# potsawee/tokenize-audio

Hardware: AMD Instinct MI355X
Metric: audio-sec encoded/sec (Mimi 8-codebook, 24 kHz) (higher is better)
Workload: dtype f16x3 (fp32-emulating: 2 fp16 planes per operand, 3 products, fp32 accumulate; RVQ distances fp32); 1 GPU; LibriTTS-R-style batch encode (configs[1]): batch=32 x 10 s @ 24 kHz resident in HBM, K=8 codebooks, 1 encode per step per GPU; global_batch=32, num_quantizers=8, parallelism=utterance round-robin x1 (no collective), gemm_precision=f16x3

## Files before the change

tokenize-audio_amd/csrc/stage0_fused.hip:

```cpp
#include <type_traits>

#include "resblock_h16.h"

namespace mimi {

#ifndef S0F_HELP
#define S0F_HELP 1
#endif
#ifndef S0F_DIAG
#define S0F_DIAG 0
#endif
#if S0F_DIAG == 3
#define S0F_DRAIN() asm volatile("" ::: "memory")
#else
#define S0F_DRAIN() asm volatile("s_waitcnt lgkmcnt(0)" ::: "memory")
#endif
namespace s0f {
constexpr int NA = 4, NC = 8, NW = NA + NC;
constexpr int YLD = 72, YSR = 36, YSS = YSR * YLD + 16, YPS = 4 * YSS, YBS = 2 * YPS;
constexpr int OFF_SLAB = r0h::NFRAG * 1024 + r0h::BIAS * 4;
constexpr int OFF_Y = OFF_SLAB + NA * r0h::WAVE_BYTES;
constexpr int OFF_D = OFF_Y + 2 * YBS * 2;
constexpr int OFF_A2 = OFF_D + 2 * NA * 16 + 16;
constexpr int LDS_BYTES = OFF_A2 + (S0F_HELP ? NA * 2 * 2 * r0h::AUD * 2 : 0);
static_assert(OFF_SLAB % 16 == 0 && OFF_Y % 16 == 0 && (YSS * 2) % 16 == 0, "16-B alignment");
static_assert(LDS_BYTES <= 160 * 1024, "LDS");
static_assert(NC * 16 == 128, "conv waves x 16 channels = down conv 0's output channels");
}

#if S0F_STAMP
#define S0F_T0() unsigned long long st_last = __builtin_readcyclecounter(), st_acc[6] = {0, 0, 0, 0, 0, 0}
#define S0F_T(i)                                                  \
    do {                                                          \
        const unsigned long long now_ = __builtin_readcyclecounter(); \
        st_acc[i] += now_ - st_last;                              \
        st_last = now_;                                           \
    } while (0)
#define S0F_TPRINT(tag)                                                                                         \
    if (blockIdx.x == 0 && lane == 0 && R > 64)                                                                 \
    printf("s0f %s wave %d rounds %d: %llu %llu %llu %llu %llu %llu\n", tag, wave, R, st_acc[0], st_acc[1],     \
           st_acc[2], st_acc[3], st_acc[4], st_acc[5])
#else
#define S0F_T0()
#define S0F_T(i)
#define S0F_TPRINT(tag)
#endif
__global__ __launch_bounds__(768) void stage0_fused_h16_kernel(ResArgs p) {
    using namespace r0h;
    constexpr int YLD = s0f::YLD, YSS = s0f::YSS, YPS = s0f::YPS, YBS = s0f::YBS, NA = s0f::NA;
    __shared__ __attribute__((aligned(16))) char lds[s0f::LDS_BYTES];
    const int tid = threadIdx.x, lane = tid & 63;
    const int wave = __builtin_amdgcn_readfirstlane(tid >> 6);
    {
        const uint4* src = reinterpret_cast<const uint4*>(p.wh16);
        uint4* dst = reinterpret_cast<uint4*>(lds);
        for (int i = tid; i < NFRAG * 64; i += s0f::NW * 64) dst[i] = src[i];
        float* bw = reinterpret_cast<float*>(lds + NFRAG * 1024);
        if (tid < 64) {
            bw[tid] = p.b0[tid];
            bw[96 + tid] = p.b1[tid];
        }
        if (tid < 32) bw[64 + tid] = p.b3[tid];
    }
    _Float16* ybase = reinterpret_cast<_Float16*>(lds + s0f::OFF_Y);
    int4* desc = reinterpret_cast<int4*>(lds + s0f::OFF_D);
    int* rcount = reinterpret_cast<int*>(lds + s0f::OFF_D + 2 * NA * 16);

    const long long T = p.T;
    const unsigned tpi = (unsigned)((T + 31) >> 5);
    const unsigned long long NT = p.istart ? p.istart[p.batch] : (unsigned long long)tpi * p.batch;
    const unsigned long long NWT = (unsigned long long)gridDim.x * NA;
    auto range = [&](int w, unsigned& g0, unsigned& g1) {
        const unsigned long long wid = (unsigned long long)blockIdx.x * NA + w;
        g0 = (unsigned)(wid * NT / NWT);
        g1 = (unsigned)((wid + 1) * NT / NWT);
    };
    if (wave < NA) {
        unsigned g0, g1;
        range(wave, g0, g1);
        TileWalk tw(p, tpi, g0);
        if (lane == 0) {
            rcount[wave] = (int)(g1 - g0) + ((g0 < g1 && tw.t0 > 0) ? 1 : 0);
            desc[NA + wave] = make_int4(0, 0, 0, 0);
        }
    }
    __syncthreads();
    int R = 0;
#pragma unroll
    for (int w = 0; w < NA; ++w) R = max(R, rcount[w]);
    const __attribute__((address_space(1))) float* __restrict__ audio =
        (const __attribute__((address_space(1))) float*)io_pointer(p.audio_ref, p.audio);
    [[maybe_unused]] _Float16* aud2 = reinterpret_cast<_Float16*>(lds + s0f::OFF_A2);

    if (wave >= NA) {
        const int co0 = 16 * (wave - NA);
        const int c16 = lane & 15, kq = lane >> 4;
        f16x8 wr[16][2];
        {
            const _Float16* wd = reinterpret_cast<const _Float16*>(p.wdown);
#pragma unroll
            for (int s = 0; s < 16; ++s) {
                const int tap = (s >> 2) + 4 * (s & 1), lo = (s >> 1) & 1;
#pragma unroll
                for (int pl = 0; pl < 2; ++pl)
                    wr[s][pl] = *reinterpret_cast<const f16x8*>(wd + (long long)(pl * 128 + co0 + c16) * 512 + tap * 64 +
                                                                32 * lo + 8 * kq);
            }
        }
        const f32x4 bd = *reinterpret_cast<const f32x4*>(p.bdown + co0 + 4 * kq);
        const float ud = p.unscale_d;
        const int sec_l = (lane >> 3) & 1, rho = lane & 7;
#if S0F_HELP
        const int hw = (wave - NA) >> 1, hrole = (wave - NA) & 1;
        unsigned hg0, hg1;
        range(hw, hg0, hg1);
        TileWalk htw(p, tpi, hg0);
        const int hhs = (hg0 < hg1 && htw.t0 > 0) ? 1 : 0;
        htw.t0 -= 32 * hhs;
        const int hRw = (int)(hg1 - hg0) + hhs;
        float mxa = 0.0f;
        auto haload = [&]() {
            const long long pos = htw.t0 - 8 + lane;
            const bool ok = lane < AUD && pos >= 0 && pos < htw.Tb;
            const float v = audio[ok ? (long long)htw.b * T + pos : 0];
            return ok ? v : 0.0f;
        };
        auto hsplit = [&](int n, float av) {
            if (lane < AUD) {
                mxa = fmaxf(mxa, fabsf(av));
                unsigned hw_, lw_;
                split2_f16s(av, 0.0f, p.ascale, hw_, lw_);
                _Float16* im = aud2 + (hw * 2 + (n & 1)) * (2 * AUD);
                im[lane] = __builtin_bit_cast(f16x2, hw_)[0];
                im[AUD + lane] = __builtin_bit_cast(f16x2, lw_)[0];
            }
        };
        const int hrow_ = (lane >> 3) & 3;
        const int hoff_ = (lane >> 5) * YPS + hw * YSS + hrow_ * YLD + 8 * ((lane & 7) ^ ((hrow_ & 1) * 2));
        float hnext = 0.0f;
        if (hrole == 0 && hRw > 0) {
            hsplit(0, haload());
            htw.next();
            if (hRw > 1) hnext = haload();
        }
        __syncthreads();
#endif
        S0F_T0();
        for (int n = 0; n <= R; ++n) {
#if S0F_HELP
            if (hrole == 1 && n < hRw) {
                uint4 v = make_uint4(0u, 0u, 0u, 0u);
                if (htw.t0 > 0) v = *reinterpret_cast<const uint4*>(ybase + ((n + 1) & 1) * YBS + hoff_ + 32 * YLD);
                *reinterpret_cast<uint4*>(ybase + (n & 1) * YBS + hoff_) = v;
                htw.next();
            }
#endif
            if (n > 0) {
                const _Float16* yb = ybase + ((n + 1) & 1) * YBS;
                const int4* dsc = desc + ((n + 1) & 1) * NA;
                f32x4 acc[2];
#pragma unroll
                for (int i = 0; i < 2; ++i) acc[i] = (f32x4){0.0f, 0.0f, 0.0f, 0.0f};
#pragma unroll
                for (int s = 0; s < 16; ++s) {
                    const int tap = (s >> 2) + 4 * (s & 1), lo = (s >> 1) & 1;
                    const int row = 4 * rho + tap, ch = 4 * lo + kq;
                    const int o = row * YLD + 8 * (ch ^ ((row & 1) * 2));
                    f16x8 yf[2][2];
#pragma unroll
                    for (int i = 0; i < 2; ++i)
#pragma unroll
                        for (int pl = 0; pl < 2; ++pl)
                            yf[pl][i] = *reinterpret_cast<const f16x8*>(yb + pl * YPS + (2 * i + sec_l) * YSS + o);
#pragma unroll
                    for (int i = 0; i < 2; ++i) {
                        if (S0F_DIAG == 1) continue;
                        acc[i] = mfma_h16(wr[s][0], yf[1][i], acc[i]);
                        acc[i] = mfma_h16(wr[s][1], yf[0][i], acc[i]);
                        acc[i] = mfma_h16(wr[s][0], yf[0][i], acc[i]);
                    }
                }
                S0F_T(0);
#pragma unroll
                for (int i = 0; i < 2; ++i) {
                    const int4 d = dsc[2 * i + sec_l];
                    if (rho < d.z) {
                        f32x4 v;
#pragma unroll
                        for (int r = 0; r < 4; ++r) v[r] = acc[i][r] * ud + bd[r];
                        *reinterpret_cast<f32x4*>(p.xout + ((long long)d.x * p.T1 + d.y + rho) * 128 + co0 + 4 * kq) = v;
                    }
                }
                S0F_T(1);
            }
#if S0F_HELP
            if (hrole == 0 && n + 1 < hRw) {
                hsplit(n + 1, hnext);
                htw.next();
                if (n + 2 < hRw) hnext = haload();
            }
#endif
            __syncthreads();
            S0F_T(2);
        }
        S0F_TPRINT("conv");
#if S0F_HELP
        amax_commit(p.aamax, mxa);
#endif
        return;
    }

#ifdef S0F_PRIO
    __builtin_amdgcn_s_setprio(S0F_PRIO);
#endif
    const f16x8* wf = reinterpret_cast<const f16x8*>(lds);
    const float* bl = reinterpret_cast<const float*>(lds + NFRAG * 1024);
    _Float16* slab = reinterpret_cast<_Float16*>(lds + s0f::OFF_SLAB + wave * WAVE_BYTES);
    _Float16* hb = slab + 2 * SLD;
    float* aud = reinterpret_cast<float*>(slab + 2 * SPL);
    unsigned g0, g1;
    range(wave, g0, g1);
    TileWalk tw(p, tpi, g0);
    const int hstart = (g0 < g1 && tw.t0 > 0) ? 1 : 0;
    tw.t0 -= 32 * hstart;
    const int Rw = (int)(g1 - g0) + hstart;
    const int j = lane & 31, hh = lane >> 5;
    const float sa = p.ascale, sx = p.xscale, sh = p.hscale, sy = p.yscale;
    const float u0 = p.unscale0, u1 = p.unscale1, u2 = p.unscale2;
    float mxa = 0.0f, mxx = 0.0f, mxh = 0.0f, mxy = 0.0f;
    auto aload = [&](unsigned bb, long long t0) {
        const long long pos = t0 - 8 + lane;
        const bool ok = lane < AUD && pos >= 0 && pos < tw.Tb;
        const float v = audio[ok ? (long long)bb * T + pos : 0];
        return ok ? v : 0.0f;
    };
    _Float16* audh = reinterpret_cast<_Float16*>(aud);
    auto conv0_img = [&](const _Float16* img, f32x16 (&x0)[2]) {
        f16x8 bq;
        const _Float16* ap = img + (hh ? AUD : 0) + j + 2;
#pragma unroll
        for (int k = 0; k < 8; ++k) bq[k] = ap[k];
#pragma unroll
        for (int mt = 0; mt < 2; ++mt) {
            f32x16 acc;
#pragma unroll
            for (int r = 0; r < 16; ++r) acc[r] = 0.0f;
            acc = mfma_h(wf[(FR_W0 + 2 * mt + 1) * 64 + lane], bq, acc);
            acc = mfma_h(wf[(FR_W0 + 2 * mt) * 64 + lane], bq, acc);
#pragma unroll
            for (int g = 0; g < 4; ++g) {
                const f32x4 bb = *reinterpret_cast<const f32x4*>(bl + 32 * mt + 8 * g + 4 * hh);
#pragma unroll
                for (int q = 0; q < 4; ++q) x0[mt][4 * g + q] = __builtin_fmaf(acc[4 * g + q], u0, bb[q]);
            }
        }
    };
    auto conv0 = [&](float av, f32x16 (&x0)[2]) {
        if (lane < AUD) {
            mxa = fmaxf(mxa, fabsf(av));
            unsigned hw, lw;
            split2_f16s(av, 0.0f, sa, hw, lw);
            audh[lane] = __builtin_bit_cast(f16x2, hw)[0];
            audh[AUD + lane] = __builtin_bit_cast(f16x2, lw)[0];
        }
        S0F_DRAIN();
        conv0_img(audh, x0);
    };
    auto slab_put = [&](const f32x16 (&x0)[2], int rowoff) {
        const int row = j + rowoff;
        if (row < 0 || row >= SROWS) return;
#pragma unroll
        for (int mt = 0; mt < 2; ++mt)
#pragma unroll
            for (int g = 0; g < 4; ++g) {
                const float z[4] = {x0[mt][4 * g], x0[mt][4 * g + 1], x0[mt][4 * g + 2], x0[mt][4 * g + 3]};
                float t[4];
                elu_s4<true>(z, sx, t, mxx);
                uint2 hi, lo;
                split4_t(t, hi, lo);
                const int o = row * SLD + 32 * mt + 8 * g + 4 * hh;
                *reinterpret_cast<uint2*>(slab + o) = hi;
                *reinterpret_cast<uint2*>(slab + SPL + o) = lo;
            }
    };
    const int cpl = lane >> 5, crow = (lane >> 4) & 1, cc = (lane & 15) * 4;
    const int hrow = (lane >> 3) & 3;
    const int hoff = (lane >> 5) * YPS + wave * YSS + hrow * YLD + 8 * ((lane & 7) ^ ((hrow & 1) * 2));
    const int yrow = 4 + j, ysw = (yrow & 1) * 2;

    if (S0F_DIAG == 2) {
        for (int i = lane; i < YSS / 8; i += 64)
#pragma unroll
            for (int q = 0; q < 4; ++q)
                *reinterpret_cast<uint4*>(ybase + q * YPS + wave * YSS + 8 * i) = make_uint4(0u, 0u, 0u, 0u);
    }
#if S0F_HELP
    __syncthreads();
#else
    float anext = Rw > 0 ? aload(tw.b, tw.t0) : 0.0f;
#endif
    S0F_T0();
    for (int n = 0; n <= R; ++n) {
        _Float16* ycur = ybase + (n & 1) * YBS;
        const _Float16* yprev = ybase + ((n + 1) & 1) * YBS;
        int4* dcur = desc + (n & 1) * NA;
        if (n < Rw && S0F_DIAG == 2) {
            if (lane == 0) dcur[wave] = make_int4((int)tw.b, (int)(tw.t0 >> 2), n < hstart ? 0 : 1, 0);
            tw.next();
        } else if (n < Rw) {
            const unsigned b = tw.b;
            const long long t0 = tw.t0;
            const long long Tb = tw.Tb;
            if (!S0F_HELP) {
                uint4 v = make_uint4(0u, 0u, 0u, 0u);
                if (t0 > 0) v = *reinterpret_cast<const uint4*>(yprev + hoff + 32 * YLD);
                *reinterpret_cast<uint4*>(ycur + hoff) = v;
            }
            if (lane == 0) {
                const long long T1b = (Tb + 3) >> 2;
                const long long t10 = t0 >> 2;
                dcur[wave] = make_int4((int)b, (int)t10, n < hstart ? 0 : (int)min(8LL, T1b - t10), 0);
            }
            if (t0 == 0) {
                *reinterpret_cast<uint2*>(slab + cpl * SPL + crow * SLD + cc) = make_uint2(0u, 0u);
            } else if (n == 0) {
                f32x16 xp[2];
                conv0(aload(b, t0 - 32), xp);
                slab_put(xp, -30);
            }
            S0F_T(0);
            f32x16 x0[2];
#if S0F_HELP
            tw.next();
            conv0_img(aud2 + (wave * 2 + (n & 1)) * (2 * AUD), x0);
#else
            const float acur = anext;
            tw.next();
            anext = aload(tw.b, tw.t0);
            conv0(acur, x0);
#endif
            S0F_T(1);
            slab_put(x0, 2);
            S0F_DRAIN();
            S0F_T(2);

            f32x16 acc1;
#pragma unroll
            for (int r = 0; r < 16; ++r) acc1[r] = 0.0f;
            f16x8 fr[2][4];
            auto g1load = [&](int ks, f16x8 (&f)[4]) {
                const int o = (j + (ks >> 2)) * SLD + (ks & 3) * 16 + 8 * hh;
                f[0] = *reinterpret_cast<const f16x8*>(slab + o);
                f[1] = *reinterpret_cast<const f16x8*>(slab + SPL + o);
                f[2] = wf[(FR_W3 + 2 * ks) * 64 + lane];
                f[3] = wf[(FR_W3 + 2 * ks + 1) * 64 + lane];
            };
            g1load(0, fr[0]);
#pragma unroll
            for (int ks = 0; ks < 12; ++ks) {
                if (ks + 1 < 12) g1load(ks + 1, fr[(ks + 1) & 1]);
                const f16x8(&f)[4] = fr[ks & 1];
                acc1 = mfma_h(f[3], f[0], acc1);
                acc1 = mfma_h(f[2], f[1], acc1);
                acc1 = mfma_h(f[2], f[0], acc1);
            }
            {
                _Float16* sp = slab + cpl * SPL;
                const uint2 v = *reinterpret_cast<const uint2*>(sp + (32 + crow) * SLD + cc);
                *reinterpret_cast<uint2*>(sp + crow * SLD + cc) = v;
            }
            asm volatile("" ::: "memory");
#pragma unroll
            for (int gq = 0; gq < 4; ++gq) {
                const f32x4 bb = *reinterpret_cast<const f32x4*>(bl + 64 + 8 * gq + 4 * hh);
                float z[4], t[4];
#pragma unroll
                for (int q = 0; q < 4; ++q) z[q] = __builtin_fmaf(acc1[4 * gq + q], u1, bb[q]);
                elu_s4<true>(z, sh, t, mxh);
                uint2 hi, lo;
                split4_t(t, hi, lo);
                const int o = j * SLD + 8 * gq + 4 * hh;
                *reinterpret_cast<uint2*>(hb + o) = hi;
                *reinterpret_cast<uint2*>(hb + SPL + o) = lo;
            }
            S0F_DRAIN();
            S0F_T(3);

            f16x8 bh[2][2];
#pragma unroll
            for (int ks = 0; ks < 2; ++ks) {
                const int o = j * SLD + ks * 16 + 8 * hh;
                bh[ks][0] = *reinterpret_cast<const f16x8*>(hb + o);
                bh[ks][1] = *reinterpret_cast<const f16x8*>(hb + SPL + o);
            }
            float tmy = 0.0f;
            const bool yin = t0 + j < Tb;
            _Float16* ys = ycur + wave * YSS + yrow * YLD + 4 * hh;
#pragma unroll
            for (int mt = 0; mt < 2; ++mt) {
                f32x16 acc2;
#pragma unroll
                for (int r = 0; r < 16; ++r) acc2[r] = 0.0f;
#pragma unroll
                for (int ks = 0; ks < 2; ++ks) {
                    const f16x8 aw0 = wf[(FR_W1 + (mt * 2 + ks) * 2) * 64 + lane];
                    const f16x8 aw1 = wf[(FR_W1 + (mt * 2 + ks) * 2 + 1) * 64 + lane];
                    acc2 = mfma_h(aw1, bh[ks][0], acc2);
                    acc2 = mfma_h(aw0, bh[ks][1], acc2);
                    acc2 = mfma_h(aw0, bh[ks][0], acc2);
                }
#pragma unroll
                for (int gq = 0; gq < 4; ++gq) {
                    const f32x4 bb = *reinterpret_cast<const f32x4*>(bl + 96 + 32 * mt + 8 * gq + 4 * hh);
                    float z[4], t[4];
#pragma unroll
                    for (int q = 0; q < 4; ++q) z[q] = x0[mt][4 * gq + q] + __builtin_fmaf(acc2[4 * gq + q], u2, bb[q]);
                    elu_s4<true>(z, sy, t, tmy);
                    uint2 hi, lo;
                    split4_t(t, hi, lo);
                    if (!yin) hi = lo = make_uint2(0u, 0u);
                    const int o = 8 * ((4 * mt + gq) ^ ysw);
                    *reinterpret_cast<uint2*>(ys + o) = hi;
                    *reinterpret_cast<uint2*>(ys + YPS + o) = lo;
                    if (p.yp && yin) {
                        _Float16* g = reinterpret_cast<_Float16*>(p.yp) + ((long long)b * T + t0 + j) * 64 + 32 * mt +
                                      8 * gq + 4 * hh;
                        *reinterpret_cast<uint2*>(g) = hi;
                        *reinterpret_cast<uint2*>(g + p.y_pstride) = lo;
                    }
                }
            }
            if (yin) mxy = fmaxf(mxy, tmy);
            S0F_T(4);
        } else if (lane == 0) {
            dcur[wave] = make_int4(0, 0, 0, 0);
        }
        __syncthreads();
        S0F_T(5);
    }
    S0F_TPRINT("block");
    amax_commit(p.aamax, mxa);
    amax_commit(p.xamax, mxx * (1.0f / sx));
    amax_commit(p.hamax, mxh * (1.0f / sh));
    amax_commit(p.yamax, mxy * (1.0f / sy));
}

hipError_t launch_stage0_fused(const ResArgs& a, hipStream_t s, const char** kname) {
    if (a.T <= 0 || a.batch <= 0 || !a.audio || !a.wh16 || !a.wdown || !a.bdown || !a.xout ||
        a.T1 != (a.T + 3) / 4)
        return hipErrorInvalidValue;
    static const char* nm = "mimi::stage0_fused_h16_kernel(mimi::ResArgs)";
    if (kname) *kname = nm;
    int dev = 0, ncu = 256;
    (void)hipGetDevice(&dev);
    (void)hipDeviceGetAttribute(&ncu, hipDeviceAttributeMultiprocessorCount, dev);
    hipLaunchKernelGGL(stage0_fused_h16_kernel, dim3((unsigned)ncu), dim3(64 * s0f::NW), 0, s, a);
    return hipGetLastError();
}

}
```

Measured before the change: 56090 audio-sec/sec.

## Software-pipeline conv0 one tile ahead and template out optional tap stores

Helper waves now split audio two tiles ahead, and each block wave computes the next tile's conv0 MFMAs interleaved with the current tile's second GEMM, carrying the result across iterations. The aim is to hide conv0 latency and LDS load latency behind the existing MFMA chain. A template parameter removes the runtime yp tap-store branch when no taps are requested. The cost is more live registers (an extra x0 accumulator set) and an added barrier at startup.

```diff
diff --git a/tokenize-audio_amd/csrc/stage0_fused.hip b/tokenize-audio_amd/csrc/stage0_fused.hip
--- a/tokenize-audio_amd/csrc/stage0_fused.hip
+++ b/tokenize-audio_amd/csrc/stage0_fused.hip
@@ -6,6 +6,16 @@
 
 #ifndef S0F_HELP
 #define S0F_HELP 1
+#endif
+#ifndef S0F_AHEAD
+#define S0F_AHEAD 1
+#endif
+#ifndef S0F_AHEAD_AT
+#define S0F_AHEAD_AT 2
+#endif
+#if !S0F_HELP
+#undef S0F_AHEAD
+#define S0F_AHEAD 0
 #endif
 #ifndef S0F_DIAG
 #define S0F_DIAG 0
@@ -26,6 +36,10 @@
 static_assert(OFF_SLAB % 16 == 0 && OFF_Y % 16 == 0 && (YSS * 2) % 16 == 0, "16-B alignment");
 static_assert(LDS_BYTES <= 160 * 1024, "LDS");
 static_assert(NC * 16 == 128, "conv waves x 16 channels = down conv 0's output channels");
+#if S0F_HELP
+static_assert(NC == 2 * NA, "S0F_HELP: two helper conv waves per block wave (audio split, y halo copy)");
+#endif
+constexpr int LEAD = S0F_AHEAD ? 2 : 1;
 }
 
 #if S0F_STAMP
@@ -45,6 +59,7 @@
 #define S0F_T(i)
 #define S0F_TPRINT(tag)
 #endif
+template <bool TAPS>
 __global__ __launch_bounds__(768) void stage0_fused_h16_kernel(ResArgs p) {
     using namespace r0h;
     constexpr int YLD = s0f::YLD, YSS = s0f::YSS, YPS = s0f::YPS, YBS = s0f::YBS, NA = s0f::NA;
@@ -137,13 +152,27 @@
         };
         const int hrow_ = (lane >> 3) & 3;
         const int hoff_ = (lane >> 5) * YPS + hw * YSS + hrow_ * YLD + 8 * ((lane & 7) ^ ((hrow_ & 1) * 2));
+        constexpr int LEAD = s0f::LEAD;
         float hnext = 0.0f;
         if (hrole == 0 && hRw > 0) {
-            hsplit(0, haload());
-            htw.next();
-            if (hRw > 1) hnext = haload();
+            float a[LEAD];
+#pragma unroll
+            for (int i = 0; i < LEAD; ++i) {
+                a[i] = 0.0f;
+                if (i < hRw) {
+                    a[i] = haload();
+                    htw.next();
+                }
+            }
+            if (hRw > LEAD) hnext = haload();
+#pragma unroll
+            for (int i = 0; i < LEAD; ++i)
+                if (i < hRw) hsplit(i, a[i]);
         }
         __syncthreads();
+#if S0F_AHEAD
+        __syncthreads();
+#endif
 #endif
         S0F_T0();
         for (int n = 0; n <= R; ++n) {
@@ -194,10 +223,10 @@
                 S0F_T(1);
             }
 #if S0F_HELP
-            if (hrole == 0 && n + 1 < hRw) {
-                hsplit(n + 1, hnext);
+            if (hrole == 0 && n + LEAD < hRw) {
+                hsplit(n + LEAD, hnext);
                 htw.next();
-                if (n + 2 < hRw) hnext = haload();
+                if (n + LEAD + 1 < hRw) hnext = haload();
             }
 #endif
             __syncthreads();
@@ -235,25 +264,36 @@
         return ok ? v : 0.0f;
     };
     _Float16* audh = reinterpret_cast<_Float16*>(aud);
-    auto conv0_img = [&](const _Float16* img, f32x16 (&x0)[2]) {
+    auto conv0_ld = [&](const _Float16* img) {
         f16x8 bq;
         const _Float16* ap = img + (hh ? AUD : 0) + j + 2;
 #pragma unroll
         for (int k = 0; k < 8; ++k) bq[k] = ap[k];
+        return bq;
+    };
+    auto conv0_mm = [&](const f16x8 bq, f32x16 (&x0)[2]) {
 #pragma unroll
         for (int mt = 0; mt < 2; ++mt) {
             f32x16 acc;
 #pragma unroll
             for (int r = 0; r < 16; ++r) acc[r] = 0.0f;
             acc = mfma_h(wf[(FR_W0 + 2 * mt + 1) * 64 + lane], bq, acc);
-            acc = mfma_h(wf[(FR_W0 + 2 * mt) * 64 + lane], bq, acc);
+            x0[mt] = mfma_h(wf[(FR_W0 + 2 * mt) * 64 + lane], bq, acc);
+        }
+    };
+    auto conv0_ep = [&](f32x16 (&x0)[2]) {
+#pragma unroll
+        for (int mt = 0; mt < 2; ++mt)
 #pragma unroll
             for (int g = 0; g < 4; ++g) {
                 const f32x4 bb = *reinterpret_cast<const f32x4*>(bl + 32 * mt + 8 * g + 4 * hh);
 #pragma unroll
-                for (int q = 0; q < 4; ++q) x0[mt][4 * g + q] = __builtin_fmaf(acc[4 * g + q], u0, bb[q]);
-            }
-        }
+                for (int q = 0; q < 4; ++q) x0[mt][4 * g + q] = __builtin_fmaf(x0[mt][4 * g + q], u0, bb[q]);
+            }
+    };
+    auto conv0_img = [&](const _Float16* img, f32x16 (&x0)[2]) {
+        conv0_mm(conv0_ld(img), x0);
+        conv0_ep(x0);
     };
     auto conv0 = [&](float av, f32x16 (&x0)[2]) {
         if (lane < AUD) {
@@ -294,8 +334,17 @@
             for (int q = 0; q < 4; ++q)
                 *reinterpret_cast<uint4*>(ybase + q * YPS + wave * YSS + 8 * i) = make_uint4(0u, 0u, 0u, 0u);
     }
+    f32x16 x0[2];
 #if S0F_HELP
     __syncthreads();
+#if S0F_AHEAD
+#pragma unroll
+    for (int mt = 0; mt < 2; ++mt)
+#pragma unroll
+        for (int r = 0; r < 16; ++r) x0[mt][r] = 0.0f;
+    if (Rw > 0) conv0_img(aud2 + wave * 2 * (2 * AUD), x0);
+    __syncthreads();
+#endif
 #else
     float anext = Rw > 0 ? aload(tw.b, tw.t0) : 0.0f;
 #endif
@@ -329,8 +378,9 @@
                 slab_put(xp, -30);
             }
             S0F_T(0);
-            f32x16 x0[2];
-#if S0F_HELP
+#if S0F_AHEAD
+            tw.next();
+#elif S0F_HELP
             tw.next();
             conv0_img(aud2 + (wave * 2 + (n & 1)) * (2 * AUD), x0);
 #else
@@ -393,28 +443,45 @@
                 bh[ks][0] = *reinterpret_cast<const f16x8*>(hb + o);
                 bh[ks][1] = *reinterpret_cast<const f16x8*>(hb + SPL + o);
             }
+#if S0F_AHEAD
+            const f16x8 bqn = conv0_ld(aud2 + (wave * 2 + ((n + (n + 1 < Rw ? 1 : 0)) & 1)) * (2 * AUD));
+            f32x16 xn[2];
+#endif
             float tmy = 0.0f;
             const bool yin = t0 + j < Tb;
             _Float16* ys = ycur + wave * YSS + yrow * YLD + 4 * hh;
-#pragma unroll
-            for (int mt = 0; mt < 2; ++mt) {
-                f32x16 acc2;
-#pragma unroll
-                for (int r = 0; r < 16; ++r) acc2[r] = 0.0f;
+            f32x16 acc2[2];
+            auto g2mm = [&](int mt) {
+#pragma unroll
+                for (int r = 0; r < 16; ++r) acc2[mt][r] = 0.0f;
 #pragma unroll
                 for (int ks = 0; ks < 2; ++ks) {
                     const f16x8 aw0 = wf[(FR_W1 + (mt * 2 + ks) * 2) * 64 + lane];
                     const f16x8 aw1 = wf[(FR_W1 + (mt * 2 + ks) * 2 + 1) * 64 + lane];
-                    acc2 = mfma_h(aw1, bh[ks][0], acc2);
-                    acc2 = mfma_h(aw0, bh[ks][1], acc2);
-                    acc2 = mfma_h(aw0, bh[ks][0], acc2);
+                    acc2[mt] = mfma_h(aw1, bh[ks][0], acc2[mt]);
+                    acc2[mt] = mfma_h(aw0, bh[ks][1], acc2[mt]);
+                    acc2[mt] = mfma_h(aw0, bh[ks][0], acc2[mt]);
                 }
+            };
+#if S0F_AHEAD && S0F_AHEAD_AT == 2
+            g2mm(0);
+            g2mm(1);
+            conv0_mm(bqn, xn);
+#endif
+#pragma unroll
+            for (int mt = 0; mt < 2; ++mt) {
+#if !(S0F_AHEAD && S0F_AHEAD_AT == 2)
+                g2mm(mt);
+#if S0F_AHEAD
+                if (mt == S0F_AHEAD_AT) conv0_mm(bqn, xn);
+#endif
+#endif
 #pragma unroll
                 for (int gq = 0; gq < 4; ++gq) {
                     const f32x4 bb = *reinterpret_cast<const f32x4*>(bl + 96 + 32 * mt + 8 * gq + 4 * hh);
                     float z[4], t[4];
 #pragma unroll
-                    for (int q = 0; q < 4; ++q) z[q] = x0[mt][4 * gq + q] + __builtin_fmaf(acc2[4 * gq + q], u2, bb[q]);
+                    for (int q = 0; q < 4; ++q) z[q] = x0[mt][4 * gq + q] + __builtin_fmaf(acc2[mt][4 * gq + q], u2, bb[q]);
                     elu_s4<true>(z, sy, t, tmy);
                     uint2 hi, lo;
                     split4_t(t, hi, lo);
@@ -422,7 +489,7 @@
                     const int o = 8 * ((4 * mt + gq) ^ ysw);
                     *reinterpret_cast<uint2*>(ys + o) = hi;
                     *reinterpret_cast<uint2*>(ys + YPS + o) = lo;
-                    if (p.yp && yin) {
+                    if (TAPS && yin) {
                         _Float16* g = reinterpret_cast<_Float16*>(p.yp) + ((long long)b * T + t0 + j) * 64 + 32 * mt +
                                       8 * gq + 4 * hh;
                         *reinterpret_cast<uint2*>(g) = hi;
@@ -431,6 +498,11 @@
                 }
             }
             if (yin) mxy = fmaxf(mxy, tmy);
+#if S0F_AHEAD
+            conv0_ep(xn);
+#pragma unroll
+            for (int mt = 0; mt < 2; ++mt) x0[mt] = xn[mt];
+#endif
             S0F_T(4);
         } else if (lane == 0) {
             dcur[wave] = make_int4(0, 0, 0, 0);
@@ -454,7 +526,10 @@
     int dev = 0, ncu = 256;
     (void)hipGetDevice(&dev);
     (void)hipDeviceGetAttribute(&ncu, hipDeviceAttributeMultiprocessorCount, dev);
-    hipLaunchKernelGGL(stage0_fused_h16_kernel, dim3((unsigned)ncu), dim3(64 * s0f::NW), 0, s, a);
+    if (a.yp)
+        hipLaunchKernelGGL(stage0_fused_h16_kernel<true>, dim3((unsigned)ncu), dim3(64 * s0f::NW), 0, s, a);
+    else
+        hipLaunchKernelGGL(stage0_fused_h16_kernel<false>, dim3((unsigned)ncu), dim3(64 * s0f::NW), 0, s, a);
     return hipGetLastError();
 }
 
```

Result: no change. 56490 audio-sec/sec, median of 6 (+0.7%).
